# lukifer23/Matrix0

Measured on NVIDIA B200. Metric: MCTS sims/sec, batched self-play, ResNet-24 (BASELINE configs[3]), higher is better.
Workload: dtype fp16

## Files before the change

### include/matrix0_b200.h

```cpp
#ifndef MATRIX0_B200_H
#define MATRIX0_B200_H

#include <stdint.h>

#ifdef __cplusplus
extern "C" {
#endif

#define M0_OK 0
#define M0_ERR_CUDA (-1)
#define M0_ERR_ARG (-2)
#define M0_ERR_STATE (-3)
#define M0_ERR_CAPACITY (-4)

#define M0_POSITION_WORDS 9
#define M0_RAW_WORDS 10
#define M0_MAX_MOVES 256
#define M0_POLICY_SIZE 4672
#define M0_PLANES 19

const char* m0_last_error(void);
int m0_version(void);
int m0_device_count(void);
int m0_device_sm_count(int device);
// ... 30 lines not shown
int m0_engine_create(int device, int max_games, int max_nodes, int tt_capacity, int max_depth, int hist_cap, m0_engine** out);
int m0_engine_destroy(m0_engine* e);
long long m0_engine_bytes(const m0_engine* e);
int m0_engine_configure(m0_engine* e, const m0_search_config* cfg, void* stream);
int m0_games_reset(m0_engine* e, const int* d_games, int n, void* stream);
int m0_games_set_positions(m0_engine* e, const int* d_games, int n, const uint64_t* d_root_pos, const uint64_t* d_hist_pos,
                           const uint16_t* d_hist_moves, const int32_t* d_hist_lens, int hist_stride, void* stream);
int m0_games_get_positions(m0_engine* e, uint64_t* d_out_pos, void* stream);
int m0_search_begin(m0_engine* e, float* d_planes, int32_t* d_info, double* d_value, void* stream);
int m0_search_select(m0_engine* e, int batch_n, float* d_planes, void* stream);
int m0_search_select_var(m0_engine* e, int batch_cap, int32_t* d_sims_left, float* d_planes, void* stream);
int m0_search_expand_backup(m0_engine* e, const float* d_logits, int logits_stride, const float* d_values, void* stream);
int m0_search_add_dirichlet(m0_engine* e, const double* d_noise, const int32_t* d_apply, void* stream);
int m0_search_pending(m0_engine* e, int32_t* d_flags_out, void* stream);
int m0_search_pending_counts(m0_engine* e, int32_t* d_counts_out, void* stream);
int m0_search_result(m0_engine* e, uint16_t* d_moves, int32_t* d_visits, double* d_child_q, double* d_prior, int32_t* d_count,
                     float* d_pi, double* d_root_q, int32_t* d_root_n, void* stream);
int m0_search_multi_enable(m0_engine* e, int samples_per_batch, int virtual_loss);
int m0_search_set_streams(m0_engine* e, const double* d_jitter, long long jitter_stride, const double* d_normal, long long normal_stride, void* stream);
int m0_search_select_multi(m0_engine* e, int batch_n, int32_t* d_sims_left, int32_t* d_row_base, int32_t* d_n_samples, void* stream);
int m0_search_multi_encode(m0_engine* e, int g0, int g1, int row0, int mode, float* d_planes, int row_cap, void* stream);
int m0_search_expand_backup_multi(m0_engine* e, int g0, int g1, const float* d_logits, int logits_stride, const float* d_values, int row0,
                                  int per_sample, int row_cap, void* stream);
int m0_engine_counters(m0_engine* e, unsigned long long* h_out16);
int m0_engine_status(m0_engine* e, int32_t* d_status_out, int32_t* d_node_count_out, void* stream);

typedef struct m0_selfplay_config {
  double temperature_start, temperature_end, resign_threshold, resign_min_entropy, resign_value_margin;
  int temperature_moves, max_game_len, min_resign_plies, resign_window, resign_consecutive_bad, opening_random_plies;
  unsigned long long seed;
  int argmax_after_plies;
  int low_visit_threshold;
  int draw_enabled, draw_min_plies, draw_window, draw_min_unique, draw_halfmove_cap, draw_material_threshold;
} m0_selfplay_config;
typedef struct m0_finished_game {
  int game, plies;
  float z;
  int reason;
  float avg_entropy;
} m0_finished_game;
int m0_selfplay_configure(m0_engine* e, const m0_selfplay_config* cfg, void* stream);
int m0_selfplay_start(m0_engine* e, void* stream);
int m0_selfplay_advance(m0_engine* e, uint16_t* d_out_move, void* stream);
int m0_selfplay_set_start_budget(m0_engine* e, long long games, void* stream);
int m0_selfplay_active_games(m0_engine* e, int* h_out, void* stream);
int m0_selfplay_set_uniforms(m0_engine* e, const double* d_uniforms);
// ... 52 lines not shown
```

### matrix0_b200/_native.py

```python
from __future__ import annotations

import ctypes
import os
from ctypes import c_char_p, c_double, c_float, c_int, c_int32, c_int64, c_uint64, c_void_p
from typing import Optional

_HERE = os.path.dirname(os.path.abspath(__file__))
LIB_PATH = os.path.join(_HERE, "_lib", "libmatrix0_b200.so")


class NativeLibraryError(RuntimeError):
    pass


_lib: Optional[ctypes.CDLL] = None

SIGNATURES = {
    "m0_last_error": (c_char_p, []),
    "m0_version": (c_int, []),
    "m0_device_count": (c_int, []),
    "m0_device_sm_count": (c_int, [c_int]),
    "m0_launch_count": (c_uint64, []),
    "m0_positions_pack": (c_int, [c_void_p, c_int, c_void_p, c_void_p]),
    "m0_random_playouts": (c_int, [c_void_p, c_int, c_uint64, c_int, c_void_p]),
# ... 1 lines not shown
    "m0_encode_planes": (c_int, [c_void_p, c_int, c_void_p, c_void_p]),
    "m0_legal_mask": (c_int, [c_void_p, c_int, c_void_p, c_void_p]),
    "m0_ssl_targets": (c_int, [c_void_p, c_int, c_void_p, c_void_p, c_void_p, c_void_p, c_void_p, c_void_p]),
    "m0_legal_moves": (c_int, [c_void_p, c_int, c_void_p, c_void_p, c_void_p, c_void_p]),
    "m0_engine_create": (c_int, [c_int, c_int, c_int, c_int, c_int, c_int, ctypes.POINTER(c_void_p)]),
    "m0_engine_destroy": (c_int, [c_void_p]),
    "m0_engine_bytes": (c_int64, [c_void_p]),
    "m0_engine_configure": (c_int, [c_void_p, c_void_p, c_void_p]),
    "m0_games_reset": (c_int, [c_void_p, c_void_p, c_int, c_void_p]),
    "m0_games_set_positions": (c_int, [c_void_p, c_void_p, c_int, c_void_p, c_void_p, c_void_p, c_void_p, c_int, c_void_p]),
    "m0_games_get_positions": (c_int, [c_void_p, c_void_p, c_void_p]),
    "m0_search_begin": (c_int, [c_void_p, c_void_p, c_void_p, c_void_p, c_void_p]),
    "m0_search_select": (c_int, [c_void_p, c_int, c_void_p, c_void_p]),
    "m0_search_expand_backup": (c_int, [c_void_p, c_void_p, c_int, c_void_p, c_void_p]),
    "m0_search_add_dirichlet": (c_int, [c_void_p, c_void_p, c_void_p, c_void_p]),
    "m0_search_pending": (c_int, [c_void_p, c_void_p, c_void_p]),
    "m0_search_pending_counts": (c_int, [c_void_p, c_void_p, c_void_p]),
    "m0_search_result": (c_int, [c_void_p, c_void_p, c_void_p, c_void_p, c_void_p, c_void_p, c_void_p, c_void_p, c_void_p, c_void_p]),
    "m0_search_multi_enable": (c_int, [c_void_p, c_int, c_int]),
    "m0_search_set_streams": (c_int, [c_void_p, c_void_p, c_int64, c_void_p, c_int64, c_void_p]),
    "m0_search_select_multi": (c_int, [c_void_p, c_int, c_void_p, c_void_p, c_void_p, c_void_p]),
    "m0_search_multi_encode": (c_int, [c_void_p, c_int, c_int, c_int, c_int, c_void_p, c_int, c_void_p]),
    "m0_search_expand_backup_multi": (c_int, [c_void_p, c_int, c_int, c_void_p, c_int, c_void_p, c_int, c_int, c_int, c_void_p]),
    "m0_engine_counters": (c_int, [c_void_p, c_void_p]),
    "m0_engine_status": (c_int, [c_void_p, c_void_p, c_void_p, c_void_p]),
    "m0_search_select_var": (c_int, [c_void_p, c_int, c_void_p, c_void_p, c_void_p]),
    "m0_selfplay_plies": (c_int, [c_void_p, c_void_p, c_void_p]),
    "m0_selfplay_configure": (c_int, [c_void_p, c_void_p, c_void_p]),
    "m0_selfplay_start": (c_int, [c_void_p, c_void_p]),
    "m0_selfplay_advance": (c_int, [c_void_p, c_void_p, c_void_p]),
    "m0_selfplay_set_start_budget": (c_int, [c_void_p, c_int64, c_void_p]),
    "m0_selfplay_active_games": (c_int, [c_void_p, ctypes.POINTER(c_int), c_void_p]),
    "m0_selfplay_set_uniforms": (c_int, [c_void_p, c_void_p]),
    "m0_trees_clear": (c_int, [c_void_p, c_void_p]),
    "m0_selfplay_finished": (c_int, [c_void_p, c_void_p, c_int, ctypes.POINTER(c_int), c_void_p]),
    "m0_net_create": (c_int, [c_int, c_void_p, c_void_p, ctypes.POINTER(c_void_p)]),
    "m0_net_destroy": (c_int, [c_void_p]),
    "m0_net_forward": (c_int, [c_void_p, c_void_p, c_int, c_void_p, c_void_p, c_int, c_void_p]),
    "m0_tc_conv": (c_int, [c_void_p, c_void_p, c_int, c_int, c_int, c_int, c_void_p, c_void_p]),
    "m0_profile_enable": (c_int, [c_int]),
    "m0_profile_get": (c_int, [c_char_p, ctypes.POINTER(c_double), ctypes.POINTER(ctypes.c_longlong)]),
    "m0_net_forward_ssl": (c_int, [c_void_p, c_void_p, c_int, c_void_p, c_void_p, c_void_p, c_void_p]),
}


class SearchConfigStruct(ctypes.Structure):
# ... 72 lines not shown
```

### matrix0_b200/arena.py

```python
from __future__ import annotations

from typing import Any, Dict, List, Optional

import numpy as np

from . import _native
from .selfplay import SelfPlayEngine


@_native.on_own_device
class _TwoEvaluatorGames(SelfPlayEngine):
    def __init__(self, model_a, model_b, *args, **kw):
        super().__init__(model_a, *args, **kw)
        import torch
        self.model_b = model_b
        self.a_is_white = torch.zeros((self.G,), dtype=torch.bool, device=self.device)
        self._pos = torch.empty((self.G, 9), dtype=torch.int64, device=self.device)
        self._ia = self._ib = None
        self.rows_a = self.rows_b = 0

    def begin_move(self) -> None:
        _native.check(self._lib.m0_games_get_positions(self.engine._h, self._pos.data_ptr(), _native.current_stream()), "m0_games_get_positions")
        white_to_move = (self._pos[:, 8] & 1).to(self.a_is_white.dtype)
        a_moves = white_to_move == self.a_is_white
        self._ia = a_moves.nonzero().squeeze(1)
        self._ib = (~a_moves).nonzero().squeeze(1)
        super().begin_move()

    def _forward(self, planes):
        import torch
        self.nn_evals += 1
        self.nn_rows += planes.shape[0]
        logits = torch.empty((self.G, 4672), dtype=torch.float32, device=self.device)
        values = torch.empty((self.G,), dtype=torch.float32, device=self.device)
# ... 59 lines not shown
```

### matrix0_b200/csrc/engine.cuh

```cuda
#pragma once
#include "m0_common.cuh"
#include "search_math.cuh"

namespace m0 {

enum { PEND_ACTIVE = 1, PEND_EXPAND = 2, PEND_REGISTER = 4, PEND_SET_Q = 8, PEND_ROOT = 16 };
enum { ST_NODE_OVERFLOW = 1, ST_TT_OVERFLOW = 2, ST_DEPTH_CAP = 4, ST_HIST_OVERFLOW = 8, ST_STREAM_EXHAUSTED = 16 };
enum { CTR_SIMS = 0, CTR_TERMINAL_SIMS, CTR_NN_EVALS, CTR_EXPANSIONS, CTR_TT_HOPS, CTR_CHILDREN_SCANNED,
       CTR_PATH_NODES, CTR_CHILDREN_CREATED, CTR_GAMES_FINISHED, CTR_POSITIONS_PLAYED, CTR_NOISY_EXPANSIONS, CTR_LEAF_SAMPLES,
       CTR_COUNT = 16 };

struct SearchParams {
  double fpu_reduction;
  double draw_penalty;
  double jitter;
  double dirichlet_alpha;
  double dirichlet_frac;
  int jitter_on;
  int no_instant_backtrack;
  int legal_softmax;
  int entropy_noise;
  int value_from_white;
  int cpuct_len;
  unsigned long long seed;
  int max_children;
  int raw_logit_priors;
  double min_child_prior;
  double virtual_loss;
  int virtual_loss_on;
  int pad_;
};

struct EngineView {
// ... 31 lines not shown
  int* pend_count;
  int* pend_flags;
  int* status;
  unsigned long long* counters;
  const SearchParams* params;
  const double* cpuct;
  const double* jit_stream;
  const double* nrm_stream;
  long long jit_stride, nrm_stride;
  unsigned long long* jit_cursor;
  unsigned long long* nrm_cursor;
  int ml_cap;
  int* ml_n_samples;
  int* ml_n_leaves;
  int* ml_smp_leaf;
  int* ml_smp_len;
  int* ml_smp_path;
  int* ml_leaf_node;
  int* ml_leaf_first;
  u64* ml_leaf_pos;
  int* ml_row_base;
  u16* node_inflight;
  double* full_scratch;
};

static constexpr u32 MOVE_NONE = 0xFFFFu;

__device__ __forceinline__ int tt_get(const EngineView& E, int g, const Key128& k) {
  const size_t base = (size_t)g * E.tt_cap;
  u32 mask = (u32)E.tt_cap - 1;
  u32 h = (u32)k.lo & mask;
  for (int probe = 0; probe < E.tt_cap; ++probe) {
    u64 lo = E.tt_lo[base + h];
    u64 hi = E.tt_hi[base + h];
    if (lo == 0 && hi == 0) return -1;
    if (lo == k.lo && hi == k.hi) return E.tt_val[base + h];
    h = (h + 1) & mask;
  }
  return -1;
}
__device__ __forceinline__ void tt_put(const EngineView& E, int g, const Key128& k, int node) {
  const size_t base = (size_t)g * E.tt_cap;
  u32 mask = (u32)E.tt_cap - 1;
  u32 h = (u32)k.lo & mask;
  for (int probe = 0; probe < E.tt_cap; ++probe) {
    u64 lo = E.tt_lo[base + h];
// ... 39 lines not shown
```

### matrix0_b200/csrc/engine_capi.cu

```cuda
#include "engine.cuh"
#include <new>
#include <string.h>

namespace m0 {
__global__ void reset_games_kernel(EngineView E, const int* games, int n_games);
__global__ void set_positions_kernel(EngineView E, const int* games, int n_games, const u64* root_pos, const u64* hist_pos,
                                     const u16* hist_moves, const int* hist_lens, int hist_stride);
__global__ void search_begin_kernel(EngineView E, float* planes, int* out_info, double* out_value);
__global__ void search_select_kernel(EngineView E, int batch_cap, int* sims_left, float* planes, unsigned long long rng_step);
__global__ void search_expand_backup_kernel(EngineView E, const float* logits, int logits_stride, const float* values);
__global__ void search_result_kernel(EngineView E, u16* out_moves, int* out_visits, double* out_child_q, double* out_prior,
                                     int* out_count, float* out_pi, double* out_root_q, int* out_root_n);
__global__ void search_add_dirichlet_kernel(EngineView E, const double* noise, const int* apply, unsigned long long rng_step);
__global__ void search_select_multi_kernel(EngineView E, int batch_cap, int* sims_left);
__global__ void multi_scan_kernel(EngineView E);
__global__ void multi_encode_kernel(EngineView E, int g0, int g1, int row0, int mode, float* planes, int row_cap);
__global__ void search_expand_backup_multi_kernel(EngineView E, int g0, int g1, const float* logits, int logits_stride, const float* values,
                                                  int row0, int per_sample, int row_cap);
}

using namespace m0;

#include "engine_host.cuh"

// ... 135 lines not shown
  dim3 grid(bx, n);
  reset_games_kernel<<<grid, 256, 0, (cudaStream_t)stream>>>(e->v, d_games, n);
  return m0_check_launch("m0_games_reset");
}

int m0_games_set_positions(m0_engine* e, const int* d_games, int n, const uint64_t* d_root_pos, const uint64_t* d_hist_pos,
                           const uint16_t* d_hist_moves, const int32_t* d_hist_lens, int hist_stride, void* stream) {
  if (!e || n < 0 || n > e->v.G || !d_root_pos) { m0_set_error("m0_games_set_positions: invalid argument"); return M0_ERR_ARG; }
  if (n == 0) return M0_OK;
  set_positions_kernel<<<n, 64, 0, (cudaStream_t)stream>>>(e->v, d_games, n, d_root_pos, d_hist_pos, d_hist_moves, d_hist_lens, hist_stride);
  return m0_check_launch("m0_games_set_positions");
}

int m0_games_get_positions(m0_engine* e, uint64_t* d_out_pos, void* stream) {
  if (!e || !d_out_pos) { m0_set_error("m0_games_get_positions: invalid argument"); return M0_ERR_ARG; }
  return m0_check_cuda(cudaMemcpyAsync(d_out_pos, e->v.root_pos, (size_t)e->v.G * 9 * sizeof(uint64_t), cudaMemcpyDeviceToDevice, (cudaStream_t)stream),
                       "m0_games_get_positions");
}

static inline int tree_blocks(const m0_engine* e) { return (e->v.G + TREE_WARPS - 1) / TREE_WARPS; }

int m0_search_begin(m0_engine* e, float* d_planes, int32_t* d_info, double* d_value, void* stream) {
  if (!e || !d_info || !d_value) { m0_set_error("m0_search_begin: invalid argument"); return M0_ERR_ARG; }
  search_begin_kernel<<<tree_blocks(e), TREE_WARPS * 32, 0, (cudaStream_t)stream>>>(e->v, d_planes, d_info, d_value);
  return m0_check_launch("m0_search_begin");
}

int m0_search_select(m0_engine* e, int batch_n, float* d_planes, void* stream) {
  if (!e || batch_n <= 0) { m0_set_error("m0_search_select: invalid argument"); return M0_ERR_ARG; }
  e->rng_step += 1;
  search_select_kernel<<<tree_blocks(e), TREE_WARPS * 32, 0, (cudaStream_t)stream>>>(e->v, batch_n, nullptr, d_planes, e->rng_step);
  return m0_check_launch("m0_search_select");
}

int m0_search_select_var(m0_engine* e, int batch_cap, int32_t* d_sims_left, float* d_planes, void* stream) {
  if (!e || batch_cap <= 0 || !d_sims_left) { m0_set_error("m0_search_select_var: invalid argument"); return M0_ERR_ARG; }
  e->rng_step += 1;
  search_select_kernel<<<tree_blocks(e), TREE_WARPS * 32, 0, (cudaStream_t)stream>>>(e->v, batch_cap, d_sims_left, d_planes, e->rng_step);
  return m0_check_launch("m0_search_select_var");
}

int m0_search_expand_backup(m0_engine* e, const float* d_logits, int logits_stride, const float* d_values, void* stream) {
  if (!e || !d_logits || !d_values || logits_stride < POLICY_SIZE) { m0_set_error("m0_search_expand_backup: invalid argument"); return M0_ERR_ARG; }
  search_expand_backup_kernel<<<tree_blocks(e), TREE_WARPS * 32, 0, (cudaStream_t)stream>>>(e->v, d_logits, logits_stride, d_values);
  return m0_check_launch("m0_search_expand_backup");
}
// ... 71 lines not shown
  if (d_row_base) M0_CUDA_TRY(cudaMemcpyAsync(d_row_base, e->v.ml_row_base, sizeof(int) * (e->v.G + 1), cudaMemcpyDeviceToDevice, s));
  if (d_n_samples) M0_CUDA_TRY(cudaMemcpyAsync(d_n_samples, e->v.ml_n_samples, sizeof(int) * e->v.G, cudaMemcpyDeviceToDevice, s));
  return M0_OK;
}

int m0_search_multi_encode(m0_engine* e, int g0, int g1, int row0, int mode, float* d_planes, int row_cap, void* stream) {
  if (!e || !d_planes || g0 < 0 || g1 > e->v.G || g0 >= g1 || e->v.ml_cap <= 0 || mode < 0 || mode > 2) { m0_set_error("m0_search_multi_encode: invalid argument"); return M0_ERR_ARG; }
  const long long warps = (long long)(g1 - g0) * e->v.ml_cap;
  multi_encode_kernel<<<(unsigned)((warps + TREE_WARPS - 1) / TREE_WARPS), TREE_WARPS * 32, 0, (cudaStream_t)stream>>>(e->v, g0, g1, row0, mode, d_planes, mode == 0 ? row_cap : 0);
  return m0_check_launch("m0_search_multi_encode");
}

int m0_search_expand_backup_multi(m0_engine* e, int g0, int g1, const float* d_logits, int logits_stride, const float* d_values, int row0,
                                  int per_sample, int row_cap, void* stream) {
  if (!e || !d_logits || !d_values || logits_stride < POLICY_SIZE || g0 < 0 || g1 > e->v.G || g0 >= g1 || e->v.ml_cap <= 0) {
    m0_set_error("m0_search_expand_backup_multi: invalid argument");
    return M0_ERR_ARG;
  }
  search_expand_backup_multi_kernel<<<(g1 - g0 + TREE_WARPS - 1) / TREE_WARPS, TREE_WARPS * 32, 0, (cudaStream_t)stream>>>(
      e->v, g0, g1, d_logits, logits_stride, d_values, row0, per_sample, per_sample ? 0 : row_cap);
  return m0_check_launch("m0_search_expand_backup_multi");
}

int m0_engine_counters(m0_engine* e, unsigned long long* h_out16) {
  if (!e || !h_out16) { m0_set_error("m0_engine_counters: invalid argument"); return M0_ERR_ARG; }
  M0_CUDA_TRY(cudaMemcpy(h_out16, e->v.counters, sizeof(unsigned long long) * CTR_COUNT, cudaMemcpyDeviceToHost));
  return M0_OK;
}
int m0_engine_status(m0_engine* e, int32_t* d_status_out, int32_t* d_node_count_out, void* stream) {
  if (!e) { m0_set_error("m0_engine_status: invalid argument"); return M0_ERR_ARG; }
  if (d_status_out) M0_CUDA_TRY(cudaMemcpyAsync(d_status_out, e->v.status, sizeof(int) * e->v.G, cudaMemcpyDeviceToDevice, (cudaStream_t)stream));
  if (d_node_count_out) M0_CUDA_TRY(cudaMemcpyAsync(d_node_count_out, e->v.node_count, sizeof(int) * e->v.G, cudaMemcpyDeviceToDevice, (cudaStream_t)stream));
  return M0_OK;
}

}
```

### matrix0_b200/csrc/tree_common.cuh

```cuda
#pragma once
#include "engine.cuh"
#include "movegen_warp.cuh"

namespace m0 {

static constexpr int TREE_WARPS = 4;
static constexpr int TREE_THREADS = TREE_WARPS * 32;
static constexpr unsigned FULL = 0xFFFFFFFFu;

__device__ __forceinline__ double uniform01(u64 x) { return (double)(x >> 11) * (1.0 / 9007199254740992.0); }

__device__ __forceinline__ double draw_jitter_uniform(const EngineView& E, const SearchParams& P, int g, unsigned long long cur, int j) {
  const unsigned long long at = cur + (unsigned long long)j;
  if (E.jit_stream && at < (unsigned long long)E.jit_stride) return E.jit_stream[(size_t)g * E.jit_stride + at];
  return uniform01(mix64(P.seed ^ mix64(0xA24BAED4963EE407ull * (u64)(g + 1)) ^ mix64(at + 0x9E3779B97F4A7C15ull)));
}
__device__ __forceinline__ double draw_noise_normal(const EngineView& E, const SearchParams& P, int g, unsigned long long cur, int j) {
  const unsigned long long at = cur + (unsigned long long)j;
  if (E.nrm_stream && at < (unsigned long long)E.nrm_stride) return E.nrm_stream[(size_t)g * E.nrm_stride + at];
  u64 a = mix64(P.seed ^ mix64(0x9FB21C651E98DF25ull * (u64)(g + 1)) ^ mix64(2 * at + 0x632BE59BD9B4E019ull));
  u64 b = mix64(a + 0x9E3779B97F4A7C15ull);
  const float u1 = ((float)(a >> 40) + 0.5f) * (1.0f / 16777216.0f), u2 = (float)(b >> 40) * (1.0f / 16777216.0f);
  return (double)(0.1f * (sqrtf(-2.0f * __logf(u1)) * __cosf(6.2831853f * u2)));
}
// ... 278 lines not shown
    E.node_w[c] = 0.0;
    E.node_q[c] = q0;
    E.node_n[c] = 0;
    E.node_first[c] = -1;
    E.node_creator[c] = node;
    E.node_mv[c] = (u32)mv | ((u32)idx[src[t]] << 16);
    E.node_nchild[c] = 0;
    if (reg) {
      Position cp = pos;
      push_move(cp, mv);
      tt_put_concurrent(E, g, position_key(cp), first + j);
    }
  }
  __syncwarp();
  if (lane == 0) {
    E.node_first[nb + node] = first;
    E.node_nchild[nb + node] = (u16)kk;
    atomicAdd(&E.counters[CTR_EXPANSIONS], 1ull);
    atomicAdd(&E.counters[CTR_CHILDREN_CREATED], (unsigned long long)kk);
  }
  __syncwarp();
}

}
```

### matrix0_b200/csrc/tree_kernels.cu

```cuda
#include "tree_common.cuh"

namespace m0 {

__global__ void reset_games_kernel(EngineView E, const int* __restrict__ games, int n_games) {
  int gi = blockIdx.y;
  if (gi >= n_games) return;
  int g = games ? games[gi] : gi;
  size_t base = (size_t)g * E.tt_cap;
  for (int i = blockIdx.x * blockDim.x + threadIdx.x; i < E.tt_cap; i += gridDim.x * blockDim.x) {
    E.tt_lo[base + i] = 0;
    E.tt_hi[base + i] = 0;
  }
  if (blockIdx.x == 0 && threadIdx.x == 0) {
    E.node_count[g] = 0;
    E.tt_count[g] = 0;
    E.hist_len[g] = 0;
    E.root_node[g] = -1;
    E.pend_flags[g] = 0;
    E.pend_count[g] = 0;
    E.status[g] = 0;
    E.active[g] = 0;
  }
}

// ... 36 lines not shown
  Key128 key = position_key(pos, &epl);
  int in_check = 0;
  int n_moves = warp_generate_legal_moves(pos, s_moves[wib], &in_check, lane);
  if (n_moves > MAX_MOVES) n_moves = MAX_MOVES;
  if (lane == 0) {
    E.root_key[g] = key;
    E.root_ep_legal[g] = epl ? 1 : 0;
    E.path_key[(size_t)g * E.max_depth] = key;
  }
  __syncwarp();
  bool terminal = n_moves == 0 || is_insufficient_material(pos) || (pos_halfmove(pos) >= 150 && n_moves > 0);
  if (!terminal && pos_halfmove(pos) >= 8) {
    int rep = 0;
    if (lane == 0) rep = leaf_is_fivefold(E, g, 0, key) ? 1 : 0;
    terminal = __shfl_sync(FULL, rep, 0) != 0;
  }
  if (terminal) {
    if (lane == 0) {
      out_info[g] = 1;
      out_value[g] = (n_moves == 0 && in_check) ? -1.0 : E.params->draw_penalty;
      E.pend_flags[g] = 0;
      E.pend_count[g] = 0;
      E.root_node[g] = -1;
    }
    return;
  }
  int root = 0, flags = 0;
  if (lane == 0) {
    root = tt_get(E, g, key);
    if (root < 0) {
      int cnt = E.node_count[g];
      if (cnt >= E.max_nodes) {
        E.status[g] |= ST_NODE_OVERFLOW;
        root = 0;
      } else {
        root = cnt;
        E.node_count[g] = cnt + 1;
        E.node_prior[nb + root] = 0.0;
        E.node_w[nb + root] = 0.0;
        E.node_q[nb + root] = 0.0;
        E.node_n[nb + root] = 0;
        E.node_first[nb + root] = -1;
        E.node_creator[nb + root] = -1;
        E.node_mv[nb + root] = MOVE_NONE;
        E.node_nchild[nb + root] = 0;
        tt_put(E, g, key, root);
// ... 4 lines not shown
    }
    E.root_node[g] = root;
    E.path_node[(size_t)g * E.max_depth] = root;
    E.path_len[g] = 1;
    E.pend_node[g] = root;
    E.pend_count[g] = 0;
    E.pend_flags[g] = flags;
    out_info[g] = flags ? 2 : 0;
    out_value[g] = 0.0;
  }
  flags = __shfl_sync(FULL, flags, 0);
  if (flags) {
    const int wtm = pos_turn(pos);
    for (int k = lane; k < n_moves; k += 32) {
      Move mv = s_moves[wib][k];
      E.leaf_moves[(size_t)g * MAX_MOVES + k] = mv;
      E.leaf_idx[(size_t)g * MAX_MOVES + k] = (u16)policy_index(mv, wtm);
    }
    if (lane == 0) {
      E.leaf_n[g] = n_moves;
      store_position(E.leaf_pos + (size_t)g * POSITION_WORDS, pos);
    }
    if (planes) warp_write_planes(pos, planes + (size_t)g * (19 * 64), lane);
  }
}

__global__ void __launch_bounds__(TREE_THREADS)
search_select_kernel(EngineView E, int batch_cap, int* __restrict__ sims_left, float* __restrict__ planes, unsigned long long rng_step) {
  __shared__ u16 s_moves[TREE_WARPS][MAX_MOVES];
  const int lane = threadIdx.x & 31, wib = threadIdx.x >> 5;
  const int g = blockIdx.x * TREE_WARPS + wib;
  if (g >= E.G || !E.active[g]) return;
  const int root = E.root_node[g];
  if (root < 0) {
    if (lane == 0) { E.pend_flags[g] = 0; E.pend_count[g] = 0; }
    return;
  }
  const SearchParams& P = *E.params;
  const size_t nb = (size_t)g * E.max_nodes;
  int* path = E.path_node + (size_t)g * E.max_depth;
  Key128* pkey = E.path_key + (size_t)g * E.max_depth;
  u8* pirrev = E.path_irrev + (size_t)g * E.max_depth;
  const Position root_pos = load_position(E.root_pos + (size_t)g * POSITION_WORDS);
  const bool root_epl = E.root_ep_legal[g] != 0;
  unsigned long long c_scanned = 0, c_path = 0, c_term = 0, c_hops = 0;

  int batch_n = batch_cap;
// ... 110 lines not shown
    E.pend_flags[g] = pend_m > 0 ? (PEND_ACTIVE | PEND_EXPAND | PEND_REGISTER) : 0;
    atomicAdd(&E.counters[CTR_SIMS], (unsigned long long)batch_n);
    atomicAdd(&E.counters[CTR_TERMINAL_SIMS], c_term);
    atomicAdd(&E.counters[CTR_CHILDREN_SCANNED], c_scanned);
    atomicAdd(&E.counters[CTR_PATH_NODES], c_path);
    atomicAdd(&E.counters[CTR_TT_HOPS], c_hops);
    if (pend_m > 0) atomicAdd(&E.counters[CTR_NN_EVALS], 1ull);
  }
}

__global__ void __launch_bounds__(TREE_THREADS)
search_expand_backup_kernel(EngineView E, const float* __restrict__ logits, int logits_stride, const float* __restrict__ values) {
  __shared__ ExpandSmem s_x[TREE_WARPS];
  const int lane = threadIdx.x & 31, wib = threadIdx.x >> 5;
  const int g = blockIdx.x * TREE_WARPS + wib;
  if (g >= E.G || !E.active[g]) return;
  const int flags = E.pend_flags[g];
  if (!(flags & PEND_ACTIVE)) return;
  const SearchParams& P = *E.params;
  const size_t nb = (size_t)g * E.max_nodes;
  const int node = E.pend_node[g];
  const int times = E.pend_count[g];
  const Position pos = load_position(E.leaf_pos + (size_t)g * POSITION_WORDS);
  float vf = values[g];
  vf = fminf(fmaxf(vf, -1.0f), 1.0f);
  double v = (double)vf;
  if ((flags & PEND_ROOT) && P.value_from_white && !pos_turn(pos)) v = -v;

  const int k = E.leaf_n[g];
  if ((flags & PEND_EXPAND) && E.node_first[nb + node] < 0 && k > 0)
    warp_expand(E, P, g, node, pos, E.leaf_moves + (size_t)g * MAX_MOVES, E.leaf_idx + (size_t)g * MAX_MOVES, k,
                logits + (size_t)g * logits_stride, (flags & PEND_REGISTER) != 0, (flags & PEND_ROOT) != 0, s_x[wib], lane);
  if ((flags & PEND_SET_Q) && lane == 0) E.node_q[nb + node] = v;
  __syncwarp();
  if (times > 0) warp_backup(E, g, E.path_len[g], py_clip_unit(v), times, lane);
  if (lane == 0) {
    E.pend_flags[g] = 0;
    E.pend_count[g] = 0;
  }
}


__device__ double gamma_variate(double alpha, u64& rng) {
  double boost = 1.0;
  if (alpha < 1.0) {
    rng = mix64(rng + 0x9E3779B97F4A7C15ull);
    double u = uniform01(rng);
    if (u <= 0.0) u = 1e-300;
    boost = pow(u, 1.0 / alpha);
    alpha += 1.0;
  }
  const double d = alpha - 1.0 / 3.0, c = 1.0 / sqrt(9.0 * d);
  for (int it = 0; it < 64; ++it) {
    rng = mix64(rng + 0x9E3779B97F4A7C15ull);
    double u1 = uniform01(rng);
// ... 95 lines not shown
```

### matrix0_b200/csrc/tree_multi_kernels.cu

```cuda
#include "tree_common.cuh"

namespace m0 {

static constexpr int WALK_CACHE_DEPTH = 12;
struct WalkCache {
  u64 pos[WALK_CACHE_DEPTH][POSITION_WORDS];
  Key128 key[WALK_CACHE_DEPTH];
  int child[WALK_CACHE_DEPTH], nxt[WALK_CACHE_DEPTH];
  u8 epl[WALK_CACHE_DEPTH], irrev[WALK_CACHE_DEPTH];
};

__global__ void __launch_bounds__(TREE_THREADS)
search_select_multi_kernel(EngineView E, int batch_cap, int* __restrict__ sims_left) {
  __shared__ u16 s_moves[TREE_WARPS][MAX_MOVES];
  __shared__ WalkCache s_cache[TREE_WARPS];
  const int lane = threadIdx.x & 31, wib = threadIdx.x >> 5;
  const int g = blockIdx.x * TREE_WARPS + wib;
  if (g >= E.G) return;
  if (!E.active[g] || E.root_node[g] < 0) {
    if (lane == 0) { E.ml_n_samples[g] = 0; E.ml_n_leaves[g] = 0; }
    return;
  }
  const int root = E.root_node[g];
  const SearchParams& P = *E.params;
// ... 224 lines not shown
  const int n_samples = E.ml_n_samples[g];
  if (n_samples <= 0) return;
  if (row_cap > 0 && E.ml_row_base[g + 1] - row0 > row_cap) return;
  const SearchParams& P = *E.params;
  const size_t nb = (size_t)g * E.max_nodes;
  const int* smp_leaf = E.ml_smp_leaf + (size_t)g * E.ml_cap;
  const int* smp_len = E.ml_smp_len + (size_t)g * E.ml_cap;
  const int* leaf_node = E.ml_leaf_node + (size_t)g * E.ml_cap;
  const int* leaf_first = E.ml_leaf_first + (size_t)g * E.ml_cap;
  const long long base = per_sample ? (long long)(g - g0) * E.ml_cap : (long long)E.ml_row_base[g] - row0;
  for (int s = 0; s < n_samples;) {
    const int r = smp_leaf[s];
    const int node = leaf_node[r];
    if (E.node_first[nb + node] < 0) {
      const Position pos = load_position(E.ml_leaf_pos + ((size_t)g * E.ml_cap + r) * POSITION_WORDS);
      int chk = 0;
      int k = warp_generate_legal_moves(pos, s_moves[wib], &chk, lane);
      if (k > MAX_MOVES) k = MAX_MOVES;
      const int wtm = pos_turn(pos);
      for (int j = lane; j < k; j += 32) s_idx[wib][j] = (u16)policy_index(s_moves[wib][j], wtm);
      __syncwarp();
      const long long lrow = base + (per_sample ? leaf_first[r] : r);
      if (k > 0) warp_expand(E, P, g, node, pos, s_moves[wib], s_idx[wib], k, logits + (size_t)lrow * logits_stride, true, false, s_x[wib], lane);
    }
    const int len = smp_len[s];
    const int* ps = E.ml_smp_path + ((size_t)g * E.ml_cap + s) * E.max_depth;
    int run = 1;
    if (!per_sample) {
      while (s + run < n_samples && smp_leaf[s + run] == r && smp_len[s + run] == len) {
        const int* pn = E.ml_smp_path + ((size_t)g * E.ml_cap + s + run) * E.max_depth;
        bool diff = false;
        for (int i = lane; i < len; i += 32) diff |= ps[i] != pn[i];
        if (__any_sync(FULL, diff)) break;
        ++run;
      }
    }
    float vf = values[base + (per_sample ? s : r)];
    vf = fminf(fmaxf(vf, -1.0f), 1.0f);
    warp_backup_path(E, g, ps, len, py_clip_unit((double)vf), run, lane);
    s += run;
  }
  if (lane == 0) {
    E.ml_n_samples[g] = 0;
    E.ml_n_leaves[g] = 0;
  }
}
// ... 3 lines not shown
```

### matrix0_b200/engine.py

```python
from __future__ import annotations

import ctypes
import math
from typing import Optional, Sequence

import numpy as np

from . import _native
from .boards import MAX_MOVES, PLANES, POLICY_SIZE, POSITION_WORDS, board_to_raw, move_to_code

COUNTER_NAMES = ["sims", "terminal_sims", "nn_evals", "expansions", "tt_hops", "children_scanned", "path_nodes",
                 "children_created", "games_finished", "positions_played", "noisy_expansions", "leaf_samples"]
ST_NODE_OVERFLOW, ST_TT_OVERFLOW, ST_DEPTH_CAP, ST_HIST_OVERFLOW, ST_STREAM_EXHAUSTED = 1, 2, 4, 8, 16


def cpuct_table(cfg, length: int) -> np.ndarray:
    out = np.empty(length, dtype=np.float64)
    for ply in range(length):
        c_base = getattr(cfg, "cpuct_c_base", None)
        c_init = getattr(cfg, "cpuct_c_init", None)
        if c_base is not None and c_init is not None:
            N = max(1.0, float(ply + 1))
            out[ply] = float(c_init) + math.log((N + float(c_base)) / float(c_base))
            continue
        start, end, span = cfg.cpuct_start, cfg.cpuct_end, int(cfg.cpuct_plies)
        if start is None or end is None or span <= 0:
            out[ply] = float(cfg.cpuct)
        else:
            t = min(max(ply, 0), span) / float(span)
            out[ply] = float(start) + (float(end) - float(start)) * t
    return out


@_native.on_own_device
class SearchEngine:
# ... 120 lines not shown
    def pending_counts(self):
        _native.check(self._lib.m0_search_pending_counts(self._h, self.pending.data_ptr(), self._stream()), "m0_search_pending_counts")
        return self.pending

    def expand_backup(self, logits, values) -> None:
        assert logits.dtype.is_floating_point and logits.element_size() == 4 and logits.is_contiguous()
        assert values.element_size() == 4 and values.is_contiguous()
        _native.check(self._lib.m0_search_expand_backup(self._h, logits.data_ptr(), logits.shape[1], values.data_ptr(), self._stream()),
                      "m0_search_expand_backup")

    def result(self, with_pi: bool = True) -> None:
        _native.check(self._lib.m0_search_result(self._h, self.res_moves.data_ptr(), self.res_visits.data_ptr(), self.res_q.data_ptr(),
                                                 self.res_prior.data_ptr(), self.res_count.data_ptr(),
                                                 self.res_pi.data_ptr() if with_pi else None, self.res_root_q.data_ptr(),
                                                 self.res_root_n.data_ptr(), self._stream()), "m0_search_result")

    def enable_multi(self, samples_per_batch: int, virtual_loss: bool = False) -> None:
        import torch
        _native.check(self._lib.m0_search_multi_enable(self._h, int(samples_per_batch), 1 if virtual_loss else 0), "m0_search_multi_enable")
        self.ml_cap = int(samples_per_batch)
        self.row_base = torch.zeros((self.G + 1,), dtype=torch.int32, device=self.device)
        self.n_samples = torch.zeros((self.G,), dtype=torch.int32, device=self.device)

    def set_streams(self, jitter=None, normal=None) -> None:
        self._streams = (jitter, normal)
        for t in (jitter, normal):
            assert t is None or (t.dtype.is_floating_point and t.element_size() == 8 and t.is_contiguous() and t.shape[0] == self.G)
        _native.check(self._lib.m0_search_set_streams(self._h, _native.ptr(jitter), 0 if jitter is None else jitter.shape[1],
                                                      _native.ptr(normal), 0 if normal is None else normal.shape[1], self._stream()),
                      "m0_search_set_streams")

    def select_multi(self, batch_n: int, sims_left=None) -> None:
        _native.check(self._lib.m0_search_select_multi(self._h, int(batch_n), _native.ptr(sims_left), self.row_base.data_ptr(),
                                                       self.n_samples.data_ptr(), self._stream()), "m0_search_select_multi")

    def multi_encode(self, g0: int, g1: int, row0: int, mode: int, planes, row_cap: int = 0) -> None:
        _native.check(self._lib.m0_search_multi_encode(self._h, int(g0), int(g1), int(row0), int(mode), planes.data_ptr(), int(row_cap),
                                                       self._stream()), "m0_search_multi_encode")

    def expand_backup_multi(self, g0: int, g1: int, logits, values, row0: int, per_sample: bool, row_cap: int = 0) -> None:
        assert logits.dtype.is_floating_point and logits.element_size() == 4 and logits.is_contiguous()
        assert values.element_size() == 4 and values.is_contiguous()
        _native.check(self._lib.m0_search_expand_backup_multi(self._h, int(g0), int(g1), logits.data_ptr(), logits.shape[1], values.data_ptr(),
                                                              int(row0), 1 if per_sample else 0, int(row_cap), self._stream()),
                      "m0_search_expand_backup_multi")

# ... 28 lines not shown
```

### matrix0_b200/selfplay.py

```python
from __future__ import annotations

import ctypes
import math
import os
import time
from typing import Any, Dict, List, Optional

import numpy as np

from . import _native
from .engine import SearchEngine
from .mcts import MCTSConfig

END_REASONS = {1: "checkmate", 2: "stalemate", 3: "insufficient_material", 4: "fifty_moves", 5: "repetition", 6: "max_game_len", 7: "resign",
               8: "draw_adjudicated"}


def resolve_draw_config(cfg_dict: Dict[str, Any]) -> Dict[str, Any]:
    merged = dict(cfg_dict.get("draw", {}) or {})
    merged.update((cfg_dict.get("selfplay", {}) or {}).get("draw", {}) or {})
    return merged


class SelfPlayConfigStruct(ctypes.Structure):
# ... 19 lines not shown
    base.setdefault("dirichlet_frac", float(sp.get("dirichlet_frac", 0.25)))
    base.setdefault("inference_batch_size", 96)
    base.setdefault("selection_jitter", float(sp.get("selection_jitter", 0.01)))
    m = dict(base)
    m.update({
        "num_simulations": int(sp.get("num_simulations", m.get("num_simulations", 800))),
        "cpuct": float(sp.get("cpuct", m.get("cpuct", 2.5))),
        "dirichlet_alpha": float(sp.get("dirichlet_alpha", m.get("dirichlet_alpha", 0.3))),
        "dirichlet_frac": float(sp.get("dirichlet_frac", m.get("dirichlet_frac", 0.25))),
        "tt_capacity": int(m.get("tt_capacity", 2000000)),
        "selection_jitter": float(sp.get("selection_jitter", m.get("selection_jitter", 0.01))),
        "inference_batch_size": int(m.get("inference_batch_size", 96)),
        "fpu": float(sp.get("fpu", m.get("fpu", 0.5))),
        "parent_q_init": bool(sp.get("parent_q_init", m.get("parent_q_init", True))),
        "tt_cleanup_frequency": int(m.get("tt_cleanup_frequency", 500)),
        "draw_penalty": float(m.get("draw_penalty", -0.1)),
        "value_from_white": bool(m.get("value_from_white", False)),
    })
    return MCTSConfig.from_dict(m)


@_native.on_own_device
class SelfPlayEngine:
    def __init__(self, model, cfg_dict: Dict[str, Any], games: int = 4096, device: Optional[int] = None, deterministic: bool = False,
                 seed: int = 1234, precision: Optional[str] = None, max_nodes: Optional[int] = None, cuda_graph: bool = True,
                 search_mode: str = "collapsed", forward_rows: Optional[int] = None):
        import torch
        if search_mode not in ("collapsed", "as_shipped", "virtual_loss"):
            raise ValueError(f"search_mode must be 'collapsed', 'as_shipped' or 'virtual_loss', got {search_mode!r}")
        self.virtual_loss = search_mode == "virtual_loss"
        self.search_mode = search_mode = "as_shipped" if self.virtual_loss else search_mode
        self.model = model
        self.cfg_dict = cfg_dict
        self.mcfg = resolve_mcts_config(cfg_dict)
        self.sp = dict(cfg_dict.get("selfplay", {}) or {})
        self.G = int(games)
        self.deterministic = bool(deterministic)
        self.precision = precision
        self.device_index = torch.cuda.current_device() if device is None else int(device)
        self.device = torch.device("cuda", self.device_index)
        bs = max(1, int(self.mcfg.inference_batch_size))
        if max_nodes is None:
            sims_hi = int(self.mcfg.num_simulations * (1.0 + max(0.0, float(self.mcfg.playout_random_frac)))) + 1
            leaves = (sims_hi if search_mode == "as_shipped" else (sims_hi + bs - 1) // bs) + 2
            max_nodes = max(4096, 1 << int(math.ceil(math.log2(leaves * 48 + 256))))
        opening = int(self.sp.get("opening_random_plies", cfg_dict.get("openings", {}).get("random_plies", 0)))
        with torch.cuda.device(self.device):
            self.engine = SearchEngine(self.G, max_nodes=max_nodes, max_depth=128,
                                       hist_cap=int(self.sp.get("max_game_len", 200)) + opening + 64, device=self.device_index)
            self.engine.configure(self.mcfg, deterministic, seed, virtual_loss=self.virtual_loss)
            if search_mode == "as_shipped":
                self.engine.enable_multi(bs, virtual_loss=self.virtual_loss)
                if forward_rows is None:
                    rnd = 4 * max(1, torch.cuda.get_device_properties(self.device).multi_processor_count // 2)
                    forward_rows = 4096 if self.virtual_loss else min(8192, max(rnd, -(-int(1.2 * self.G) // rnd) * rnd))
                self.forward_rows = max(bs, min(int(forward_rows), self.G * bs))
                self.forward_rows += self.forward_rows & 1
                self.forward_sizes = sorted({self.forward_rows} | {s for s in (256, 512, 1024, 2048) if bs <= s < self.forward_rows})
                self.ml_planes = torch.zeros((self.forward_rows, 19, 8, 8), dtype=torch.float32, device=self.device)
            s = SelfPlayConfigStruct()
            s.temperature_start = float(self.sp.get("temperature_start", 1.0))
            s.temperature_end = float(self.sp.get("temperature_end", 0.1))
            s.temperature_moves = int(self.sp.get("temperature_moves", 20))
            s.resign_threshold = float(self.sp.get("resign_threshold", -0.98))
            s.resign_min_entropy = float(self.sp.get("resign_min_entropy", 0.3))
            s.resign_value_margin = float(self.sp.get("resign_value_margin", 0.05))
            s.max_game_len = int(self.sp.get("max_game_len", 200))
            s.min_resign_plies = int(self.sp.get("min_resign_plies", 24))
            s.resign_window = int(self.sp.get("resign_window", 4))
            s.resign_consecutive_bad = int(self.sp.get("resign_consecutive_bad", 5))
            s.opening_random_plies = int(self.sp.get("opening_random_plies", cfg_dict.get("openings", {}).get("random_plies", 0)))
            s.seed = int(seed) & 0xFFFFFFFFFFFFFFFF
            s.argmax_after_plies = int(self.sp.get("argmax_after_plies", -1))
            s.low_visit_threshold = int(self.sp.get("low_visit_threshold", 0) or 0)
            draw = resolve_draw_config(cfg_dict)
            s.draw_enabled = 1 if bool(draw.get("enabled", False)) else 0
            s.draw_min_plies = int(draw.get("min_plies", 30))
            s.draw_window = int(draw.get("window", 12))
            s.draw_min_unique = int(draw.get("min_unique", 3))
            s.draw_halfmove_cap = int(draw.get("halfmove_cap", 50))
            s.draw_material_threshold = int(draw.get("material_draw_threshold", 10))
            lib = _native.lib()
# ... 50 lines not shown
        if self.cuda_graph and (self.precision or getattr(self.model, "precision", "fp32")) != "fp32":
            key = (planes.data_ptr(), planes.shape[0], self.model.ws_epoch)
            if key not in self._graphs:
                lib = _native.lib()
                self._graphs = {k: v for k, v in self._graphs.items() if k[2] == self.model.ws_epoch}
                g, lg, v = self.model.capture_forward(planes, self.precision)
                if self.model.ws_epoch != key[2]:
                    self._graphs = {}
                    key = (planes.data_ptr(), planes.shape[0], self.model.ws_epoch)
                n0 = int(lib.m0_launch_count())
                self.model.forward_planes(planes, self.precision)
                self.graph_kernels = int(lib.m0_launch_count()) - n0
                self._graphs[key] = (g, lg, v)
            g, lg, v = self._graphs[key]
            g.replay()
            self.graph_replays += 1
            return lg, v
        return self.model.forward_planes(planes, self.precision) if self.precision else self.model.forward_planes(planes)

    def begin_move(self) -> None:
        import torch
        eng = self.engine
        _native.check(self._lib.m0_trees_clear(eng._h, _native.current_stream()), "m0_trees_clear")
        eng.begin()
        logits, values = self._forward(eng.planes)
        eng.expand_backup(logits, values)
        if not self.deterministic and float(self.mcfg.dirichlet_frac) > 0:
            _native.check(self._lib.m0_selfplay_plies(eng._h, self.plies.data_ptr(), _native.current_stream()), "m0_selfplay_plies")
            dp = getattr(self.mcfg, "dirichlet_plies", None)
            apply = None if dp is None else (self.plies < int(dp)).to(torch.int32)
            eng.add_dirichlet(None, apply)
        sims = int(self.mcfg.num_simulations)
        frac = 0.0 if self.deterministic else float(self.mcfg.playout_random_frac)
        if frac > 0.0 and sims > 0:
            low = int(max(1, sims * (1.0 - frac)))
            high = int(max(low, sims * (1.0 + frac)))
            self.sims_left.copy_(torch.randint(low, high + 1, (self.G,), device=self.device, generator=self._gen, dtype=torch.int32))
        else:
            self.sims_left.fill_(sims)
        self.steps += 1

    def search_step(self) -> None:
        eng = self.engine
        if self.search_mode == "as_shipped":
            return self._search_step_as_shipped()
        ev = self.tree_events
        if ev is not None:
            import torch
            e = [torch.cuda.Event(enable_timing=True) for _ in range(4)]
            e[0].record()
        _native.check(self._lib.m0_search_select_var(eng._h, int(self.mcfg.inference_batch_size), self.sims_left.data_ptr(),
                                                     eng.planes.data_ptr(), _native.current_stream()), "m0_search_select_var")
        if ev is not None:
            e[1].record()
        logits, values = self._forward(eng.planes)
        if ev is not None:
            e[2].record()
        eng.expand_backup(logits, values)
        if ev is not None:
            e[3].record()
            ev.append(e)
        self.steps += 1

    def warm_up_forward(self) -> None:
        if self.search_mode != "as_shipped":
            return
        for size in sorted(self.forward_sizes, reverse=True):
            self._forward(self.ml_planes[:size])
        self.nn_evals = self.nn_rows = 0

    def _search_step_as_shipped(self) -> None:
        eng = self.engine
        eng.select_multi(int(self.mcfg.inference_batch_size), self.sims_left)
        G, cap = self.G, self.forward_rows
        planes = self.ml_planes[:cap]
        eng.multi_encode(0, G, 0, 0, planes, row_cap=cap)
        logits, values = self._forward(planes)
        eng.expand_backup_multi(0, G, logits, values, 0, per_sample=False, row_cap=cap)
        rb = eng.row_base.cpu().numpy()
        g0 = max(int(np.searchsorted(rb, cap, side="right")) - 1, 0)
        self.nn_rows += int(rb[g0]) - cap
        self.nn_rows_padded += cap
        while g0 < G:
            g1 = int(np.searchsorted(rb, rb[g0] + cap, side="right")) - 1
            g1 = min(max(g1, g0 + 1), G)
            rows = int(rb[g1] - rb[g0])
            if rows > 0:
                size = next(s for s in self.forward_sizes if s >= rows)
                planes = self.ml_planes[:size]
                eng.multi_encode(g0, g1, int(rb[g0]), 0, planes)
                logits, values = self._forward(planes)
# ... 144 lines not shown
```

Baseline: 12.36 million.

## Reuse cached depth-1 child evaluations for next move's root network eval

Adds a per-game cache of network logits and values for root children expanded during search. At the next move, if the new root position matches a cached child, its evaluation is reused and only missed roots are compacted into a smaller batch for the forward pass. This saves root-eval network work each move, at the cost of copying a full policy row on every depth-1 expansion, a host sync on the miss count, and extra CUDA graph sizes.

```diff
diff --git a/include/matrix0_b200.h b/include/matrix0_b200.h
--- a/include/matrix0_b200.h
+++ b/include/matrix0_b200.h
@@ -76,6 +76,8 @@
 int m0_search_multi_encode(m0_engine* e, int g0, int g1, int row0, int mode, float* d_planes, int row_cap, void* stream);
 int m0_search_expand_backup_multi(m0_engine* e, int g0, int g1, const float* d_logits, int logits_stride, const float* d_values, int row0,
                                   int per_sample, int row_cap, void* stream);
+int m0_search_reuse_enable(m0_engine* e, int slots, float* d_miss_planes, int32_t* d_miss_count);
+int m0_search_reuse_clear(m0_engine* e, void* stream);
 int m0_engine_counters(m0_engine* e, unsigned long long* h_out16);
 int m0_engine_status(m0_engine* e, int32_t* d_status_out, int32_t* d_node_count_out, void* stream);
 
diff --git a/matrix0_b200/_native.py b/matrix0_b200/_native.py
--- a/matrix0_b200/_native.py
+++ b/matrix0_b200/_native.py
@@ -47,6 +47,8 @@
     "m0_search_select_multi": (c_int, [c_void_p, c_int, c_void_p, c_void_p, c_void_p, c_void_p]),
     "m0_search_multi_encode": (c_int, [c_void_p, c_int, c_int, c_int, c_int, c_void_p, c_int, c_void_p]),
     "m0_search_expand_backup_multi": (c_int, [c_void_p, c_int, c_int, c_void_p, c_int, c_void_p, c_int, c_int, c_int, c_void_p]),
+    "m0_search_reuse_enable": (c_int, [c_void_p, c_int, c_void_p, c_void_p]),
+    "m0_search_reuse_clear": (c_int, [c_void_p, c_void_p]),
     "m0_engine_counters": (c_int, [c_void_p, c_void_p]),
     "m0_engine_status": (c_int, [c_void_p, c_void_p, c_void_p, c_void_p]),
     "m0_search_select_var": (c_int, [c_void_p, c_int, c_void_p, c_void_p, c_void_p]),
diff --git a/matrix0_b200/arena.py b/matrix0_b200/arena.py
--- a/matrix0_b200/arena.py
+++ b/matrix0_b200/arena.py
@@ -10,6 +10,8 @@
 
 @_native.on_own_device
 class _TwoEvaluatorGames(SelfPlayEngine):
+    reuse_root_evals = False
+
     def __init__(self, model_a, model_b, *args, **kw):
         super().__init__(model_a, *args, **kw)
         import torch
diff --git a/matrix0_b200/csrc/engine.cuh b/matrix0_b200/csrc/engine.cuh
--- a/matrix0_b200/csrc/engine.cuh
+++ b/matrix0_b200/csrc/engine.cuh
@@ -8,7 +8,8 @@
 enum { ST_NODE_OVERFLOW = 1, ST_TT_OVERFLOW = 2, ST_DEPTH_CAP = 4, ST_HIST_OVERFLOW = 8, ST_STREAM_EXHAUSTED = 16 };
 enum { CTR_SIMS = 0, CTR_TERMINAL_SIMS, CTR_NN_EVALS, CTR_EXPANSIONS, CTR_TT_HOPS, CTR_CHILDREN_SCANNED,
        CTR_PATH_NODES, CTR_CHILDREN_CREATED, CTR_GAMES_FINISHED, CTR_POSITIONS_PLAYED, CTR_NOISY_EXPANSIONS, CTR_LEAF_SAMPLES,
-       CTR_COUNT = 16 };
+       CTR_ROOT_REUSED, CTR_COUNT = 16 };
+static constexpr int REUSE_MAX_SLOTS = 64;
 
 struct SearchParams {
   double fpu_reduction;
@@ -86,6 +87,14 @@
   int* ml_row_base;
   u16* node_inflight;
   double* full_scratch;
+  int rc_slots;
+  int* rc_fill;
+  u64* rc_pos;
+  float* rc_logits;
+  float* rc_value;
+  int* rc_src;
+  float* rc_miss_planes;
+  int* rc_miss_count;
 };
 
 static constexpr u32 MOVE_NONE = 0xFFFFu;
diff --git a/matrix0_b200/csrc/engine_capi.cu b/matrix0_b200/csrc/engine_capi.cu
--- a/matrix0_b200/csrc/engine_capi.cu
+++ b/matrix0_b200/csrc/engine_capi.cu
@@ -181,6 +181,7 @@
 
 int m0_search_begin(m0_engine* e, float* d_planes, int32_t* d_info, double* d_value, void* stream) {
   if (!e || !d_info || !d_value) { m0_set_error("m0_search_begin: invalid argument"); return M0_ERR_ARG; }
+  if (e->v.rc_slots) M0_CUDA_TRY(cudaMemsetAsync(e->v.rc_miss_count, 0, sizeof(int), (cudaStream_t)stream));
   search_begin_kernel<<<tree_blocks(e), TREE_WARPS * 32, 0, (cudaStream_t)stream>>>(e->v, d_planes, d_info, d_value);
   return m0_check_launch("m0_search_begin");
 }
@@ -298,6 +299,31 @@
   return m0_check_launch("m0_search_expand_backup_multi");
 }
 
+int m0_search_reuse_enable(m0_engine* e, int slots, float* d_miss_planes, int32_t* d_miss_count) {
+  if (!e || slots <= 0 || slots > REUSE_MAX_SLOTS || !d_miss_planes || !d_miss_count) { m0_set_error("m0_search_reuse_enable: invalid argument"); return M0_ERR_ARG; }
+  if (e->v.rc_slots && e->v.rc_slots != slots) { m0_set_error("m0_search_reuse_enable: already enabled with %d slots", e->v.rc_slots); return M0_ERR_STATE; }
+  EngineView& v = e->v;
+  if (!v.rc_slots) {
+    m0::DeviceGuard device_guard(e->device);
+    M0_CUDA_TRY(device_guard.err);
+    const size_t G = v.G, S = G * (size_t)slots;
+    TRY(dev_alloc(e, &v.rc_fill, G));
+    TRY(dev_alloc(e, &v.rc_pos, S * POSITION_WORDS, false));
+    TRY(dev_alloc(e, &v.rc_logits, S * POLICY_SIZE, false));
+    TRY(dev_alloc(e, &v.rc_value, S, false));
+    TRY(dev_alloc(e, &v.rc_src, G, false));
+    v.rc_slots = slots;
+  }
+  v.rc_miss_planes = d_miss_planes;
+  v.rc_miss_count = d_miss_count;
+  return M0_OK;
+}
+
+int m0_search_reuse_clear(m0_engine* e, void* stream) {
+  if (!e || !e->v.rc_slots) { m0_set_error("m0_search_reuse_clear: invalid argument (store not enabled)"); return M0_ERR_ARG; }
+  return m0_check_cuda(cudaMemsetAsync(e->v.rc_fill, 0, sizeof(int) * e->v.G, (cudaStream_t)stream), "m0_search_reuse_clear");
+}
+
 int m0_engine_counters(m0_engine* e, unsigned long long* h_out16) {
   if (!e || !h_out16) { m0_set_error("m0_engine_counters: invalid argument"); return M0_ERR_ARG; }
   M0_CUDA_TRY(cudaMemcpy(h_out16, e->v.counters, sizeof(unsigned long long) * CTR_COUNT, cudaMemcpyDeviceToHost));
diff --git a/matrix0_b200/csrc/tree_common.cuh b/matrix0_b200/csrc/tree_common.cuh
--- a/matrix0_b200/csrc/tree_common.cuh
+++ b/matrix0_b200/csrc/tree_common.cuh
@@ -324,4 +324,27 @@
   __syncwarp();
 }
 
-}
+__device__ __forceinline__ void warp_record_root_child(const EngineView& E, int g, const u64* pos_words, const float* __restrict__ lg,
+                                                       float value, int lane) {
+  const int n = E.rc_fill[g];
+  if (n >= E.rc_slots) return;
+  const size_t e = (size_t)g * E.rc_slots + n;
+  float* dst = E.rc_logits + e * POLICY_SIZE;
+  if ((reinterpret_cast<uintptr_t>(lg) & 15) == 0) {
+    const float4* s4 = reinterpret_cast<const float4*>(lg);
+    float4* d4 = reinterpret_cast<float4*>(dst);
+#pragma unroll 4
+    for (int i = lane; i < POLICY_SIZE / 4; i += 32) d4[i] = __ldg(s4 + i);
+  } else {
+    for (int i = lane; i < POLICY_SIZE; i += 32) dst[i] = lg[i];
+  }
+  if (lane < POSITION_WORDS) E.rc_pos[e * POSITION_WORDS + lane] = pos_words[lane];
+  __syncwarp();
+  if (lane == 0) {
+    E.rc_value[e] = value;
+    E.rc_fill[g] = n + 1;
+  }
+  __syncwarp();
+}
+
+}
diff --git a/matrix0_b200/csrc/tree_kernels.cu b/matrix0_b200/csrc/tree_kernels.cu
--- a/matrix0_b200/csrc/tree_kernels.cu
+++ b/matrix0_b200/csrc/tree_kernels.cu
@@ -82,6 +82,7 @@
       E.pend_flags[g] = 0;
       E.pend_count[g] = 0;
       E.root_node[g] = -1;
+      if (E.rc_slots) E.rc_fill[g] = 0;
     }
     return;
   }
@@ -132,7 +133,33 @@
       store_position(E.leaf_pos + (size_t)g * POSITION_WORDS, pos);
     }
     if (planes) warp_write_planes(pos, planes + (size_t)g * (19 * 64), lane);
-  }
+    if (E.rc_slots) {
+      const u64* rw = E.root_pos + (size_t)g * POSITION_WORDS;
+      const int fill = E.rc_fill[g];
+      int src = 0;
+      bool hit = false;
+      for (int e0 = 0; e0 < fill && !hit; e0 += 32) {
+        const u64* ew = E.rc_pos + ((size_t)g * E.rc_slots + e0 + lane) * POSITION_WORDS;
+        bool eq = e0 + lane < fill;
+        for (int w = 0; w < POSITION_WORDS && eq; ++w) eq = ew[w] == rw[w];
+        const unsigned hits = __ballot_sync(FULL, eq);
+        if (hits) {
+          hit = true;
+          src = -1 - (e0 + __ffs(hits) - 1);
+        }
+      }
+      if (hit) {
+        if (lane == 0) atomicAdd(&E.counters[CTR_ROOT_REUSED], 1ull);
+      } else {
+        int row = 0;
+        if (lane == 0) row = atomicAdd(E.rc_miss_count, 1);
+        src = __shfl_sync(FULL, row, 0);
+        warp_write_planes(pos, E.rc_miss_planes + (size_t)src * (19 * 64), lane);
+      }
+      if (lane == 0) E.rc_src[g] = src;
+    }
+  }
+  if (E.rc_slots && lane == 0) E.rc_fill[g] = 0;
 }
 
 __global__ void __launch_bounds__(TREE_THREADS)
@@ -289,7 +316,23 @@
   const int node = E.pend_node[g];
   const int times = E.pend_count[g];
   const Position pos = load_position(E.leaf_pos + (size_t)g * POSITION_WORDS);
-  float vf = values[g];
+  const float* lg;
+  float vf;
+  if ((flags & PEND_ROOT) && E.rc_slots) {
+    const int src = E.rc_src[g];
+    if (src < 0) {
+      const size_t e = (size_t)g * E.rc_slots + (-1 - src);
+      lg = E.rc_logits + e * POLICY_SIZE;
+      vf = E.rc_value[e];
+    } else {
+      lg = logits + (size_t)src * logits_stride;
+      vf = values[src];
+    }
+  } else {
+    lg = logits + (size_t)g * logits_stride;
+    vf = values[g];
+    if (E.rc_slots && E.path_len[g] == 2) warp_record_root_child(E, g, E.leaf_pos + (size_t)g * POSITION_WORDS, lg, vf, lane);
+  }
   vf = fminf(fmaxf(vf, -1.0f), 1.0f);
   double v = (double)vf;
   if ((flags & PEND_ROOT) && P.value_from_white && !pos_turn(pos)) v = -v;
@@ -297,7 +340,7 @@
   const int k = E.leaf_n[g];
   if ((flags & PEND_EXPAND) && E.node_first[nb + node] < 0 && k > 0)
     warp_expand(E, P, g, node, pos, E.leaf_moves + (size_t)g * MAX_MOVES, E.leaf_idx + (size_t)g * MAX_MOVES, k,
-                logits + (size_t)g * logits_stride, (flags & PEND_REGISTER) != 0, (flags & PEND_ROOT) != 0, s_x[wib], lane);
+                lg, (flags & PEND_REGISTER) != 0, (flags & PEND_ROOT) != 0, s_x[wib], lane);
   if ((flags & PEND_SET_Q) && lane == 0) E.node_q[nb + node] = v;
   __syncwarp();
   if (times > 0) warp_backup(E, g, E.path_len[g], py_clip_unit(v), times, lane);
diff --git a/matrix0_b200/csrc/tree_multi_kernels.cu b/matrix0_b200/csrc/tree_multi_kernels.cu
--- a/matrix0_b200/csrc/tree_multi_kernels.cu
+++ b/matrix0_b200/csrc/tree_multi_kernels.cu
@@ -270,6 +270,9 @@
       __syncwarp();
       const long long lrow = base + (per_sample ? leaf_first[r] : r);
       if (k > 0) warp_expand(E, P, g, node, pos, s_moves[wib], s_idx[wib], k, logits + (size_t)lrow * logits_stride, true, false, s_x[wib], lane);
+      if (E.rc_slots && smp_len[s] == 2)
+        warp_record_root_child(E, g, E.ml_leaf_pos + ((size_t)g * E.ml_cap + r) * POSITION_WORDS, logits + (size_t)lrow * logits_stride,
+                               values[lrow], lane);
     }
     const int len = smp_len[s];
     const int* ps = E.ml_smp_path + ((size_t)g * E.ml_cap + s) * E.max_depth;
diff --git a/matrix0_b200/engine.py b/matrix0_b200/engine.py
--- a/matrix0_b200/engine.py
+++ b/matrix0_b200/engine.py
@@ -10,7 +10,7 @@
 from .boards import MAX_MOVES, PLANES, POLICY_SIZE, POSITION_WORDS, board_to_raw, move_to_code
 
 COUNTER_NAMES = ["sims", "terminal_sims", "nn_evals", "expansions", "tt_hops", "children_scanned", "path_nodes",
-                 "children_created", "games_finished", "positions_played", "noisy_expansions", "leaf_samples"]
+                 "children_created", "games_finished", "positions_played", "noisy_expansions", "leaf_samples", "root_evals_reused"]
 ST_NODE_OVERFLOW, ST_TT_OVERFLOW, ST_DEPTH_CAP, ST_HIST_OVERFLOW, ST_STREAM_EXHAUSTED = 1, 2, 4, 8, 16
 
 
@@ -177,6 +177,16 @@
         self.row_base = torch.zeros((self.G + 1,), dtype=torch.int32, device=self.device)
         self.n_samples = torch.zeros((self.G,), dtype=torch.int32, device=self.device)
 
+    def enable_reuse(self, slots: int) -> None:
+        import torch
+        self.miss_planes = torch.zeros((self.G, PLANES, 8, 8), dtype=torch.float32, device=self.device)
+        self.miss_count = torch.zeros((1,), dtype=torch.int32, device=self.device)
+        _native.check(self._lib.m0_search_reuse_enable(self._h, int(slots), self.miss_planes.data_ptr(), self.miss_count.data_ptr()),
+                      "m0_search_reuse_enable")
+
+    def clear_reuse(self) -> None:
+        _native.check(self._lib.m0_search_reuse_clear(self._h, self._stream()), "m0_search_reuse_clear")
+
     def set_streams(self, jitter=None, normal=None) -> None:
         self._streams = (jitter, normal)
         for t in (jitter, normal):
diff --git a/matrix0_b200/selfplay.py b/matrix0_b200/selfplay.py
--- a/matrix0_b200/selfplay.py
+++ b/matrix0_b200/selfplay.py
@@ -65,6 +65,8 @@
 
 @_native.on_own_device
 class SelfPlayEngine:
+    reuse_root_evals = True
+
     def __init__(self, model, cfg_dict: Dict[str, Any], games: int = 4096, device: Optional[int] = None, deterministic: bool = False,
                  seed: int = 1234, precision: Optional[str] = None, max_nodes: Optional[int] = None, cuda_graph: bool = True,
                  search_mode: str = "collapsed", forward_rows: Optional[int] = None):
@@ -101,6 +103,12 @@
                 self.forward_rows += self.forward_rows & 1
                 self.forward_sizes = sorted({self.forward_rows} | {s for s in (256, 512, 1024, 2048) if bs <= s < self.forward_rows})
                 self.ml_planes = torch.zeros((self.forward_rows, 19, 8, 8), dtype=torch.float32, device=self.device)
+            if self.reuse_root_evals:
+                self.engine.enable_reuse(32 if search_mode == "as_shipped" else min(32, self.batches_per_move()))
+                self.root_sizes = sorted({self.G} | {s for s in (256, 512, 1024, 2048) if s < self.G})
+                self._no_rows = (torch.zeros((1, 4672), dtype=torch.float32, device=self.device),
+                                 torch.zeros((1,), dtype=torch.float32, device=self.device))
+                self._reuse_epoch = model.ws_epoch
             s = SelfPlayConfigStruct()
             s.temperature_start = float(self.sp.get("temperature_start", 1.0))
             s.temperature_end = float(self.sp.get("temperature_end", 0.1))
@@ -197,8 +205,21 @@
         import torch
         eng = self.engine
         _native.check(self._lib.m0_trees_clear(eng._h, _native.current_stream()), "m0_trees_clear")
-        eng.begin()
-        logits, values = self._forward(eng.planes)
+        if not self.reuse_root_evals:
+            eng.begin()
+            logits, values = self._forward(eng.planes)
+        else:
+            if self.model.ws_epoch != self._reuse_epoch:
+                eng.clear_reuse()
+                self._reuse_epoch = self.model.ws_epoch
+            eng.begin()
+            n = int(eng.miss_count.item())
+            if n:
+                size = next(s for s in self.root_sizes if s >= n)
+                logits, values = self._forward(eng.miss_planes[:size])
+                self.nn_rows += n - size
+            else:
+                logits, values = self._no_rows
         eng.expand_backup(logits, values)
         if not self.deterministic and float(self.mcfg.dirichlet_frac) > 0:
             _native.check(self._lib.m0_selfplay_plies(eng._h, self.plies.data_ptr(), _native.current_stream()), "m0_selfplay_plies")
@@ -238,10 +259,11 @@
         self.steps += 1
 
     def warm_up_forward(self) -> None:
-        if self.search_mode != "as_shipped":
-            return
-        for size in sorted(self.forward_sizes, reverse=True):
-            self._forward(self.ml_planes[:size])
+        calls = [(self.ml_planes, s) for s in self.forward_sizes] if self.search_mode == "as_shipped" else []
+        if self.reuse_root_evals:
+            calls += [(self.engine.miss_planes, s) for s in self.root_sizes]
+        for buf, size in sorted(calls, key=lambda c: -c[1]):
+            self._forward(buf[:size])
         self.nn_evals = self.nn_rows = 0
 
     def _search_step_as_shipped(self) -> None:
```

After: 13.75 million, median of 6. 11.3% higher.
